# rneddojr/Adapting-Pretrained-Vision-Transformers-with-LoRA-against-Attack-Vectors

Hardware: AMD Instinct MI355X
Metric: adversarial images/sec (PGD-20, ViT-B/16+LoRA r=8, bs256) (higher is better)
Workload: dtype f16; 1 GPU; PGD-20 eps=8/255 alpha=2/255 random_start, ViT-B/16 (21 classes) + LoRA r=8 on q,k,v,attn-out,fc2 (fused), batch 256/GPU of synthetic 224x224x3 in HBM, seeded random-init weights; global_batch=256, per_gpu_batch=256, scaling=weak, pgd_steps=20, lora_rank=8, parallelism=dp1 (batch shards, no data-path collective), ranks_seen_by_collective=1

## Files before the change

adapting-pretrained-vision-transformers-with-lora-against-attack-vectors_amd/csrc/attention32.hip:

```cpp
#include <cstdlib>
#include <cstring>
#include <type_traits>

#include "env.h"
#include "kernels.h"
#include "prof.h"

namespace VLNS {

#ifdef VITLORA_ATTN_STAMPS
__device__ unsigned long long g_attn_stamps[8192 * 8 * 8];
#define STAMP(k) do { if (blockIdx.x < 8192 && (threadIdx.x & 63) == 0) g_attn_stamps[(blockIdx.x * 8 + (threadIdx.x >> 6)) * 8 + (k)] = __builtin_amdgcn_s_memtime(); } while (0)
#define ISTAMP(hd, k) do { if ((hd) == 3) { __builtin_amdgcn_sched_barrier(0); unsigned long long t_; asm volatile("s_memtime %0\n\ts_waitcnt lgkmcnt(0)" : "=s"(t_) :: "memory"); __builtin_amdgcn_sched_barrier(0); if (blockIdx.x < 1024 && (threadIdx.x & 63) == 0) g_attn_stamps[(blockIdx.x * 8 + (threadIdx.x >> 6)) * 8 + (k)] = t_; } } while (0)
#else
#define STAMP(k) do { } while (0)
#define ISTAMP(hd, k) do { } while (0)
#endif
#ifdef VITLORA_ATTN_STAMPS_FWD
#undef ISTAMP
#define ISTAMP(hd, k) do { } while (0)
#define FSTAMP(hd, k) do { if ((hd) == 3) { __builtin_amdgcn_sched_barrier(0); unsigned long long t_; asm volatile("s_memtime %0\n\ts_waitcnt lgkmcnt(0)" : "=s"(t_) :: "memory"); __builtin_amdgcn_sched_barrier(0); if (blockIdx.x < 1024 && (threadIdx.x & 63) == 0) g_attn_stamps[(blockIdx.x * 8 + (threadIdx.x >> 6)) * 8 + (k)] = t_; } } while (0)
#else
#define FSTAMP(hd, k) do { } while (0)
#endif
#ifdef VITLORA_ATTN_STAMPS2
#undef ISTAMP
#define ISTAMP(hd, k) do { } while (0)
#define JSTAMP(hd, i, k) do { if ((hd) == 3 && (i) == 3) { __builtin_amdgcn_sched_barrier(0); unsigned long long t_; asm volatile("s_memtime %0\n\ts_waitcnt lgkmcnt(0)" : "=s"(t_) :: "memory"); __builtin_amdgcn_sched_barrier(0); if (blockIdx.x < 1024 && (threadIdx.x & 63) == 0) g_attn_stamps[(blockIdx.x * 8 + (threadIdx.x >> 6)) * 8 + (k)] = t_; } } while (0)
#else
#define JSTAMP(hd, i, k) do { } while (0)
#endif

#define LDS_BARRIER()                                                        \
    do {                                                                     \
        __builtin_amdgcn_sched_barrier(0);                                   \
        asm volatile("s_waitcnt lgkmcnt(0)\n\ts_barrier" ::: "memory");       \
        __builtin_amdgcn_sched_barrier(0);                                   \
    } while (0)

namespace {

#ifndef VL_ATTN_NT
#define VL_ATTN_NT 0
#endif
__device__ __forceinline__ void glds16a(const void* gsrc, void* lds_wave_base) {
    __builtin_amdgcn_global_load_lds(GLB_PTR(gsrc), LDS_PTR(lds_wave_base), 16, 0, VL_ATTN_NT ? 2 : 0);
}
__device__ __forceinline__ h16x8 ld_attn(const h16* p) {
#if VL_ATTN_NT
    return __builtin_nontemporal_load((const h16x8*)p);
#else
    return *(const h16x8*)p;
#endif
}



constexpr int HD = 64;
#define TPAD(t) ((double)(((t) + 31) / 32 * 32))
typedef float f32x16 __attribute__((ext_vector_type(16)));
typedef float f32x2 __attribute__((ext_vector_type(2)));

__device__ __forceinline__ f32x16 mfma32(h16x8 a, h16x8 b, f32x16 c) {
#ifdef VL_BF16
    return __builtin_amdgcn_mfma_f32_32x32x16_bf16(a, b, c, 0, 0, 0);
#else
    return __builtin_amdgcn_mfma_f32_32x32x16_f16(a, b, c, 0, 0, 0);
#endif
}
__device__ __forceinline__ float fexp2(float x) { return __builtin_amdgcn_exp2f(x); }
__device__ __forceinline__ int swz(int r) { return (((r >> 1) & 1) << 2) | ((r >> 2) & 3); }

__device__ __forceinline__ h16x8 row_frag32(const h16* img, int row, int ks, int h) {
    return *(const h16x8*)(img + row * HD + (((2 * ks + h) ^ swz(row)) << 3));
}
__device__ __forceinline__ h16x8 tr_frag32(const h16* img, int t0, int c0, int lane) {
    const int g = lane >> 4, i = lane & 15;
    const int h = g >> 1, q = i >> 2, p = i & 3;
    const int col = c0 + 16 * (g & 1) + 4 * p;
    const int r0 = t0 + 4 * h + q, r1 = r0 + 8;
    const h16* a0 = img + r0 * HD + (((col >> 3) ^ swz(r0)) << 3) + (col & 4);
    const h16* a1 = img + r1 * HD + (((col >> 3) ^ swz(r1)) << 3) + (col & 4);
    return cat4(lds_read_tr16(a0), lds_read_tr16(a1));
}
__device__ __forceinline__ h16x8 pack8(const f32x16& v, int s) {
    h16x8 o;
#pragma unroll
    for (int j = 0; j < 8; ++j) o[j] = f2h(v[8 * s + j]);
    return o;
}
struct FragOffs {
    int row[4];
    int tr[2][2];
};
__device__ __forceinline__ FragOffs frag_offs(int lane) {
    FragOffs o;
    const int c = lane & 31, h = lane >> 5;
#pragma unroll
    for (int ks = 0; ks < 4; ++ks) o.row[ks] = c * HD + (((2 * ks + h) ^ swz(c)) << 3);
    const int g = lane >> 4, i = lane & 15;
    const int th = g >> 1, q = i >> 2, p = i & 3;
#pragma unroll
    for (int dt = 0; dt < 2; ++dt)
#pragma unroll
        for (int e = 0; e < 2; ++e) {
            const int r = 4 * th + q + 8 * e;
            o.tr[dt][e] = r * HD + (((dt * 4 + 2 * (g & 1) + (p >> 1)) ^ swz(r)) << 3) + ((p & 1) << 2);
        }
    return o;
}
__device__ __forceinline__ h16x8 row_frag_o(const h16* img, int tile, int off) {
    return *(const h16x8*)(img + tile * 32 * HD + off);
}
__device__ __forceinline__ h16x8 tr_frag_o(const h16* img, int tile, int st, const int (&off)[2]) {
    const h16* b = img + tile * 32 * HD + st * 16 * HD;
    return cat4(lds_read_tr16(b + off[0]), lds_read_tr16(b + off[1]));
}
template <int ROWS, int NW>
__device__ __forceinline__ void stage_glds(h16* img, const h16* src, int ld, int T, int w, int lane) {
    const int lr = lane >> 3, lc = lane & 7;
#pragma unroll 1
    for (int g = w; g < ROWS / 8; g += NW) {
        const int r = g * 8 + lr;
        const int rs = r < T ? r : T - 1;
        glds16a(src + (size_t)rs * ld + ((lc ^ swz(r)) << 3), img + g * 8 * HD);
    }
}

__device__ __forceinline__ void store_rows32_half(char* img, const f32x16 (&acc)[2], float mul, h16* dst0, int ld, int tok0,
                                                  int T, int lane) {
    const int c = lane & 31, h = lane >> 5;
    const int lr = lane >> 3, lc = lane & 7;
#pragma unroll
    for (int p = 0; p < 2; ++p) {
        if ((c >> 4) == p) {
#pragma unroll
            for (int dt = 0; dt < 2; ++dt)
#pragma unroll
                for (int rq = 0; rq < 4; ++rq) {
                    h16x4 o;
#pragma unroll
                    for (int k = 0; k < 4; ++k) o[k] = f2h(acc[dt][4 * rq + k] * mul);
                    *(h16x4*)(img + (c & 15) * 128 + (((dt * 4 + rq) ^ (c & 7)) << 4) + 8 * h) = o;
                }
        }
#pragma unroll
        for (int ps = 0; ps < 2; ++ps) {
            const int row = ps * 8 + lr;
            const h16x8 v = *(const h16x8*)(img + row * 128 + ((lc ^ lr) << 4));
            const int tok = tok0 + p * 16 + row;
            if (tok < T) *(h16x8*)(dst0 + (size_t)tok * ld + lc * 8) = v;
        }
    }
}

constexpr int FWD_WAVES = 8;
template <int NT>
__global__ __launch_bounds__(64 * FWD_WAVES) void attn_fwd32_kernel(const h16* __restrict__ qkv, h16* __restrict__ ctx,
                                                            float* __restrict__ lse2, int T, int H, int D, float scale_log2e) {
    constexpr int ROWS = NT * 32;
    __shared__ __attribute__((aligned(16))) h16 sm[2 * ROWS * HD];
    __shared__ __attribute__((aligned(16))) char wimg[FWD_WAVES * 2048];
    h16* sK = sm;
    h16* sV = sm + ROWS * HD;
    const int tid = threadIdx.x, lane = tid & 63;
    const int w = __builtin_amdgcn_readfirstlane(tid >> 6);
    const int c = lane & 31, h = lane >> 5;
    const int b = blockIdx.x / H, hd = blockIdx.x - b * H;
    const int ld = 3 * D;
    const h16* base = qkv + (size_t)b * T * ld + hd * HD;
    stage_glds<ROWS, FWD_WAVES>(sK, base + D, ld, T, w, lane);
    stage_glds<ROWS, FWD_WAVES>(sV, base + 2 * D, ld, T, w, lane);

    const int nqb = (T + 31) >> 5;
    int qb = w;
    h16x8 qf[4];
    auto load_q = [&](int blk) {
        const int q = blk * 32 + c;
        const h16* qr = base + (size_t)(q < T ? q : T - 1) * ld + 8 * h;
#pragma unroll
        for (int ks = 0; ks < 4; ++ks) qf[ks] = *(const h16x8*)(qr + 16 * ks);
    };
    if (qb < nqb) load_q(qb);
    asm volatile("s_waitcnt vmcnt(0)" ::: "memory");
    __syncthreads();

    const FragOffs fo = frag_offs(lane);
    const int tcut = T - 4 * h;
    for (; qb < nqb; qb += FWD_WAVES) {
        float m = -INFINITY, l = 0.f;
        f32x16 o[2];
#pragma unroll
        for (int dt = 0; dt < 2; ++dt)
#pragma unroll
            for (int r = 0; r < 16; ++r) o[dt][r] = 0.f;
        auto step = [&](int kt, auto masked) {
            constexpr bool MASKED = decltype(masked)::value;
            f32x16 s;
#pragma unroll
// ... 594 lines not shown
            auto stepA = [&](int kt, auto masked) {
                constexpr bool MASKED = decltype(masked)::value;
                f32x16 s, dp;
#pragma unroll
                for (int r = 0; r < 16; ++r) { s[r] = 0.f; dp[r] = 0.f; }
#pragma unroll
                for (int ks = 0; ks < 4; ++ks) {
                    s = mfma32(row_frag_o(sK, kt, fo.row[ks]), fa[ks], s);
                    dp = mfma32(row_frag_o(sV, kt, fo.row[ks]), fb[ks], dp);
                }
#pragma unroll
                for (int r = 0; r < 16; r += 2) {
                    const f32x2 t = f32x2{s[r], s[r + 1]} * f32x2{scale_log2e, scale_log2e} - f32x2{lse_q, lse_q};
                    f32x2 p = {fexp2(t[0]), fexp2(t[1])};
                    if constexpr (MASKED) {
                        if (kt * 32 + (r & 3) + 8 * (r >> 2) >= tcut) p[0] = 0.f;
                        if (kt * 32 + ((r + 1) & 3) + 8 * ((r + 1) >> 2) >= tcut) p[1] = 0.f;
                    }
                    const f32x2 d = p * (f32x2{dp[r], dp[r + 1]} - f32x2{delta_q, delta_q});
                    dp[r] = d[0]; dp[r + 1] = d[1];
                }
#pragma unroll
                for (int st = 0; st < 2; ++st) {
                    const h16x8 dsb = pack8(dp, st);
#pragma unroll
                    for (int dt = 0; dt < 2; ++dt) dq[dt] = mfma32(tr_frag_o(sK, kt, st, fo.tr[dt]), dsb, dq[dt]);
                }
            };
            const int nfull = T >> 5;
#pragma unroll 1
            for (int kt = 0; kt < nfull; ++kt) stepA(kt, std::false_type{});
            if (T & 31) stepA(nfull, std::true_type{});
            ISTAMP(hd, 1);
#pragma unroll
            for (int ks = 0; ks < 4; ++ks) { fa[ks] = row_frag32(sK, tok, ks, h); fb[ks] = row_frag32(sV, tok, ks, h); }
#pragma unroll
            for (int dt = 0; dt < 2; ++dt)
#pragma unroll
                for (int r = 0; r < 16; ++r) dq[dt][r] *= scale;
            if (lo.W && (lo.mods & 1u)) {
                f32x16 y;
#pragma unroll
                for (int r = 0; r < 16; ++r) y[r] = 0.f;
                const h16* sB = sBd + (hd & 1) * 3 * 8 * HD;
#pragma unroll
                for (int dt = 0; dt < 2; ++dt)
#pragma unroll
                    for (int st = 0; st < 2; ++st) y = mfma32(down_frag_lds(sB, dt, st, lane), pack8(dq[dt], st), y);
                down_accumulate(usum, y, tok, h);
            }
            store_rows32_half(wimg + w * 2048, dq, 1.f, dqkv + (size_t)b * T * ld + hd * HD, ld, w * 32, T, lane);
        }
        ISTAMP(hd, 2);
        LDS_BARRIER();
        ISTAMP(hd, 3);
        if (loader) {
            if (hd + 1 < H) {
                stage_glds<ROWS, 1>(sK, base + D + (hd + 1) * HD, ld, T, 0, lane);
                stage_glds<ROWS, 1>(sV, base + 2 * D + (hd + 1) * HD, ld, T, 0, lane);
                if (lo.W) stage_bd(hd + 1);
            }
            asm volatile("s_waitcnt vmcnt(0)" ::: "memory");
        } else if (active) {
            f32x16 dv[2], dk[2];
#pragma unroll
            for (int dt = 0; dt < 2; ++dt)
#pragma unroll
                for (int r = 0; r < 16; ++r) { dv[dt][r] = 0.f; dk[dt][r] = 0.f; }
#pragma unroll 1
            for (int qt = 0; qt < nb; ++qt) {
                f32x16 s, dp;
#pragma unroll
                for (int r = 0; r < 16; ++r) { s[r] = 0.f; dp[r] = 0.f; }
#pragma unroll
                for (int ks = 0; ks < 4; ++ks) {
                    s = mfma32(row_frag_o(sQ, qt, fo.row[ks]), fa[ks], s);
                    dp = mfma32(row_frag_o(sdO, qt, fo.row[ks]), fb[ks], dp);
                }
#pragma unroll
                for (int rq = 0; rq < 4; ++rq) {
                    const f32x4 lq = *(const f32x4*)(L + qt * 32 + 8 * rq + 4 * h);
                    const f32x4 dl = *(const f32x4*)(Dl + qt * 32 + 8 * rq + 4 * h);
#pragma unroll
                    for (int k = 0; k < 4; ++k) {
                        const float p = fexp2(fmaf(s[4 * rq + k], scale_log2e, -lq[k]));
                        s[4 * rq + k] = p;
                        dp[4 * rq + k] = p * (dp[4 * rq + k] - dl[k]);
                    }
                }
#pragma unroll
                for (int st = 0; st < 2; ++st) {
                    const h16x8 pb = pack8(s, st), dsb = pack8(dp, st);
#pragma unroll
                    for (int dt = 0; dt < 2; ++dt) {
                        dv[dt] = mfma32(tr_frag_o(sdO, qt, st, fo.tr[dt]), pb, dv[dt]);
                        dk[dt] = mfma32(tr_frag_o(sQ, qt, st, fo.tr[dt]), dsb, dk[dt]);
                    }
                }
            }
            ISTAMP(hd, 4);
#pragma unroll
            for (int dt = 0; dt < 2; ++dt)
#pragma unroll
                for (int r = 0; r < 16; ++r) dk[dt][r] *= scale;
            if (lo.W) {
                const h16* sB = sBd + (hd & 1) * 3 * 8 * HD;
#pragma unroll
                for (int md = 1; md < 3; ++md) {
                    if (!((lo.mods >> md) & 1u)) continue;
                    f32x16 y;
#pragma unroll
                    for (int r = 0; r < 16; ++r) y[r] = 0.f;
#pragma unroll
                    for (int dt = 0; dt < 2; ++dt)
#pragma unroll
                        for (int st = 0; st < 2; ++st)
                            y = mfma32(down_frag_lds(sB + md * 8 * HD, dt, st, lane), pack8(md == 1 ? dk[dt] : dv[dt], st), y);
                    down_accumulate(usum + md * ROWS * 8, y, tok, h);
                }
            }
            store_rows32_half(wimg + w * 2048, dk, 1.f, dqkv + (size_t)b * T * ld + D + hd * HD, ld, w * 32, T, lane);
            store_rows32_half(wimg + w * 2048, dv, 1.f, dqkv + (size_t)b * T * ld + 2 * D + hd * HD, ld, w * 32, T, lane);
            ISTAMP(hd, 7);
            if (hd + 1 < H) fetch_a(hd + 1);
        }
        ISTAMP(hd, 5);
        LDS_BARRIER();
        ISTAMP(hd, 6);
    }
    if (lo.W && !loader && active && tok < T && 4 * h < lo.r) {
        h16* dst = lo.out + ((size_t)b * T + tok) * 64 + 4 * h;
#pragma unroll
        for (int md = 0; md < 3; ++md) {
            if (!((lo.mods >> md) & 1u)) continue;
            const f32x4 u4 = *(const f32x4*)(usum + (md * ROWS + tok) * 8 + 4 * h);
            h16x4 v;
#pragma unroll
            for (int k = 0; k < 4; ++k) v[k] = f2h(u4[k]);
            *(h16x4*)(dst + md * lo.r) = v;
        }
    }
}

#ifndef RING_PRIO
#define RING_PRIO 0
#endif
template <int NT> constexpr int ring_img_rows() { return NT == 7 ? 200 : NT * 32; }
template <int NT>
size_t bwd_ring_lds() {
    return (size_t)4 * ring_img_rows<NT>() * HD * sizeof(h16) + (size_t)2 * NT * 2048 + (size_t)4 * NT * 32 * sizeof(float) +
           (size_t)3 * NT * 32 * 8 * sizeof(float) + (size_t)2 * 3 * 8 * HD * sizeof(h16);
}

template <int NT>
__global__ __launch_bounds__(64 * IMG_WAVES) void attn_bwd_ring_kernel(const h16* __restrict__ qkv, const h16* __restrict__ ctx,
                                                                       const h16* __restrict__ dctx, const float* __restrict__ lse2,
                                                                       h16* __restrict__ dqkv, int T, int H, int D, float scale,
                                                                       float scale_log2e, const LoraDown lo) {
    constexpr int ROWS = NT * 32, IR = ring_img_rows<NT>();
    extern __shared__ __attribute__((aligned(16))) char smem[];
    h16* sQ = (h16*)smem;
    h16* sdO = sQ + IR * HD;
    h16* sK0 = sdO + IR * HD;
    char* sE = (char*)(sK0 + 2 * IR * HD);
    float* sLD = (float*)(sE + 2 * NT * 2048);
    float* usum = sLD + 4 * ROWS;
    h16* sBd = (h16*)(usum + 3 * ROWS * 8);

    const int tid = threadIdx.x, lane = tid & 63;
    const int w = __builtin_amdgcn_readfirstlane(tid >> 6);
    const int c = lane & 31, h = lane >> 5;
    const int b = blockIdx.x;
    const int ld = 3 * D;
    const h16* base = qkv + (size_t)b * T * ld;
    const h16* dobase = dctx + (size_t)b * T * D;
    const h16* obase = ctx + (size_t)b * T * D;
    const int nb = (T + 31) >> 5;

    for (int i = tid; i < 3 * ROWS * 8; i += 64 * IMG_WAVES) usum[i] = 0.f;
    for (int i = tid; i < 2 * NT * 2048 / 16; i += 64 * IMG_WAVES) ((f32x4*)sE)[i] = f32x4{0.f, 0.f, 0.f, 0.f};
    if constexpr (ROWS > IR)
        for (int i = tid; i < (ROWS - IR) * HD * 2 / 16; i += 64 * IMG_WAVES) ((f32x4*)(sK0 + IR * HD))[i] = f32x4{0.f, 0.f, 0.f, 0.f};

    if (w == IMG_WAVES - 1) {
        h16x8 bdv[3];
        auto bd_issue = [&](int hd) {
            const int j = lane >> 3, c8 = (lane & 7) * 8;
#pragma unroll
            for (int md = 0; md < 3; ++md) {
#pragma unroll
                for (int k = 0; k < 8; ++k) bdv[md][k] = (h16)0.f;
                if (((lo.mods >> md) & 1u) && j < lo.r) bdv[md] = *(const h16x8*)(lo.W + (size_t)(md * lo.r + j) * ld + md * D + hd * HD + c8);
            }
        };
        auto bd_commit = [&](int hd) {
            const int j = lane >> 3, c8 = (lane & 7) * 8;
            h16* dst = sBd + (hd & 1) * 3 * 8 * HD;
#pragma unroll
            for (int md = 0; md < 3; ++md) *(h16x8*)(dst + md * 8 * HD + j * HD + c8) = bdv[md];
        };
        h16x8 rd8[4], ro8[4];
        float rlse = 0.f;
        auto consts_issue = [&](int hd, int blk) {
            const int t = blk * 32 + c, tc = t < T ? t : T - 1;
#pragma unroll
            for (int ks = 0; ks < 4; ++ks) {
                rd8[ks] = ld_attn(dobase + (size_t)tc * D + hd * HD + 8 * h + 16 * ks);
                ro8[ks] = ld_attn(obase + (size_t)tc * D + hd * HD + 8 * h + 16 * ks);
            }
            rlse = lse2[((size_t)b * H + hd) * T + tc];
        };
        auto consts_finish = [&](int hd, int blk) {
            const int t = blk * 32 + c;
            float delta_q = 0.f;
#pragma unroll
            for (int ks = 0; ks < 4; ++ks)
#pragma unroll
                for (int k = 0; k < 8; ++k) delta_q = fmaf(h2f(rd8[ks][k]), h2f(ro8[ks][k]), delta_q);
            delta_q += __shfl_xor(delta_q, 32, 64);
            if (h == 0) {
                float* Lw = sLD + (hd & 1) * 2 * ROWS;
                Lw[t] = t < T ? rlse : INFINITY;
                Lw[ROWS + t] = t < T ? delta_q : 0.f;
            }
        };
        stage_glds<IR, 1>(sQ, base, ld, T, 0, lane);
        stage_glds<IR, 1>(sdO, dobase, D, T, 0, lane);
        stage_glds<IR, 1>(sK0, base + D, ld, T, 0, lane);
        if (lo.W) {
            h16x8 z;
#pragma unroll
            for (int k = 0; k < 8; ++k) z[k] = (h16)0.f;
            for (int i = lane; i < T * 8; i += 64) *(h16x8*)(lo.out + ((size_t)b * T + (i >> 3)) * 64 + (i & 7) * 8) = z;
            bd_issue(0);
            bd_commit(0);
        }
        for (int blk = 0; blk < NT; ++blk) { consts_issue(0, blk); consts_finish(0, blk); }
        asm volatile("s_waitcnt vmcnt(0)" ::: "memory");
        LDS_BARRIER();
#pragma unroll 1
        for (int hd = 0; hd < H; ++hd) {
            const bool more = hd + 1 < H;
            ISTAMP(hd, 0);
            if (more) {
                consts_issue(hd + 1, 0);
                if (lo.W) bd_issue(hd + 1);
            }
#pragma unroll 1
            for (int i = 0; i < nb; ++i) {
                if (i == 3) ISTAMP(hd, 1);
                if (more) {
                    consts_finish(hd + 1, i);
                    if (i == 0 && lo.W) bd_commit(hd + 1);
                    if (i + 1 < NT) consts_issue(hd + 1, i + 1);
                    {
                        constexpr int NG = IR / 8;
                        const int per = (NG + nb - 1) / nb;
                        const int lr = lane >> 3, lc = lane & 7;
                        h16* img = sK0 + ((hd + 1) & 1) * IR * HD;
                        const h16* src = base + D + (hd + 1) * HD;
                        for (int g = i * per; g < (i + 1) * per && g < NG; ++g) {
                            const int r = g * 8 + lr;
                            const int rs = r < T ? r : T - 1;
                            glds16a(src + (size_t)rs * ld + ((lc ^ swz(r)) << 3), img + g * 8 * HD);
                        }
                    }
                }
                if (i == nb - 1) {
                    if (more) for (int blk = nb; blk < NT; ++blk) { consts_finish(hd + 1, blk); if (blk + 1 < NT) consts_issue(hd + 1, blk + 1); }
                    asm volatile("s_waitcnt vmcnt(0)" ::: "memory");
                }
                if (i == 3) ISTAMP(hd, 2);
                LDS_BARRIER();
                if (i == 3) ISTAMP(hd, 3);
            }
            ISTAMP(hd, 4);
            if (more) {
                stage_glds<IR, 1>(sQ, base + (hd + 1) * HD, ld, T, 0, lane);
                stage_glds<IR, 1>(sdO, dobase + (hd + 1) * HD, D, T, 0, lane);
            }
            asm volatile("s_waitcnt vmcnt(0)" ::: "memory");
            ISTAMP(hd, 6);
            LDS_BARRIER();
            ISTAMP(hd, 7);
        }
        return;
    }
    if (w >= nb) {
        LDS_BARRIER();
        for (int hd = 0; hd < H; ++hd) {
            for (int i = 0; i < nb; ++i) LDS_BARRIER();
            LDS_BARRIER();
        }
        return;
    }
    const FragOffs fo = frag_offs(lane);
    const int tok = w * 32 + c, tokc = tok < T ? tok : T - 1;
    int ewr[2], erd[2];
    {
        const int f = (c >> 2) & 3;
#pragma unroll
        for (int r1 = 0; r1 < 2; ++r1) ewr[r1] = c * 64 + (((2 * r1 + h) ^ f) << 3);
        const int g = lane >> 4, i16 = lane & 15, q4 = i16 >> 2, p4 = i16 & 3;
#pragma unroll
        for (int e = 0; e < 2; ++e) {
            const int r = 4 * (g >> 1) + q4 + 8 * e;
            erd[e] = r * 64 + (((4 * (g & 1) + p4) ^ ((r >> 2) & 3)) << 3);
        }
    }
    h16x8 fb[4];
#pragma unroll
    for (int ks = 0; ks < 4; ++ks) fb[ks] = ld_attn(base + (size_t)tokc * ld + 2 * D + 8 * h + 16 * ks);
    if (w >= 4 && RING_PRIO) __builtin_amdgcn_s_setprio(1);
    LDS_BARRIER();

#pragma unroll 1
    for (int hd = 0; hd < H; ++hd) {
        const h16* sK = sK0 + (hd & 1) * IR * HD;
        const float* L = sLD + (hd & 1) * 2 * ROWS;
        const float* Dl = L + ROWS;
        f32x16 dq[2], dk[2], dv[2];
#pragma unroll
        for (int dt = 0; dt < 2; ++dt)
#pragma unroll
            for (int r = 0; r < 16; ++r) { dq[dt][r] = 0.f; dk[dt][r] = 0.f; dv[dt][r] = 0.f; }
        h16x8 pbk[2], dsk[2];
#pragma unroll
        for (int st = 0; st < 2; ++st)
#pragma unroll
            for (int j = 0; j < 8; ++j) { pbk[st][j] = (h16)0.f; dsk[st][j] = (h16)0.f; }
        int qp = w, kp = w;
        ISTAMP(hd, 0);
        auto take_ds = [&](int step, int kt_, int st) -> h16x8 {
            const char* eslot = sE + ((step & 1) * NT + w) * 2048;
            h16x8 d = cat4(lds_read_tr16(eslot + 1024 * st + erd[0]), lds_read_tr16(eslot + 1024 * st + erd[1]));
            if (kt_ == nb - 1 && (T & 31)) {
#pragma unroll
                for (int j = 0; j < 8; ++j)
                    if (kt_ * 32 + 16 * st + 8 * (j >> 2) + 4 * h + (j & 3) >= T) d[j] = (h16)0.f;
            }
            return d;
        };
#pragma unroll 1
        for (int i = 0; i < nb; ++i) {
            int qt = w + i; if (qt >= nb) qt -= nb;
            int kt = w - i; if (kt < 0) kt += nb;
            if (i == 3) ISTAMP(hd, 1);
            JSTAMP(hd, i, 0);
            f32x16 s, dp;
#pragma unroll
            for (int r = 0; r < 16; ++r) { s[r] = 0.f; dp[r] = 0.f; }
#pragma unroll
            for (int ks = 0; ks < 4; ++ks) s = mfma32(row_frag_o(sQ, qt, fo.row[ks]), row_frag_o(sK, w, fo.row[ks]), s);
#pragma unroll
            for (int ks = 0; ks < 4; ++ks) dp = mfma32(row_frag_o(sdO, qt, fo.row[ks]), fb[ks], dp);
            h16x8 fv0[2], fk0[2], fv1[2], fk1[2], fq0[2], fq1[2], d0, d1;
#pragma unroll
            for (int dt = 0; dt < 2; ++dt) { fv0[dt] = tr_frag_o(sdO, qp, 0, fo.tr[dt]); fk0[dt] = tr_frag_o(sQ, qp, 0, fo.tr[dt]); }
            __builtin_amdgcn_sched_barrier(0);
            JSTAMP(hd, i, 1);
            char* eslot_w = sE + ((i & 1) * NT + qt) * 2048;
            auto exp_piece = [&](int rq) {
                const f32x4 lq = *(const f32x4*)(L + qt * 32 + 8 * rq + 4 * h);
                const f32x4 dl = *(const f32x4*)(Dl + qt * 32 + 8 * rq + 4 * h);
                h16x4 ds4;
#pragma unroll
                for (int k = 0; k < 4; ++k) {
                    const float p = fexp2(fmaf(s[4 * rq + k], scale_log2e, -lq[k]));
                    const float d = p * (dp[4 * rq + k] - dl[k]);
                    pbk[rq >> 1][4 * (rq & 1) + k] = f2h(p);
                    ds4[k] = f2h_sat(d);
                    dsk[rq >> 1][4 * (rq & 1) + k] = ds4[k];
                }
                *(h16x4*)(eslot_w + ewr[rq & 1] + 32 * (rq >> 1)) = ds4;
            };
#pragma unroll
            for (int dt = 0; dt < 2; ++dt) { fv1[dt] = tr_frag_o(sdO, qp, 1, fo.tr[dt]); fk1[dt] = tr_frag_o(sQ, qp, 1, fo.tr[dt]); }
#pragma unroll
            for (int dt = 0; dt < 2; ++dt) { dv[dt] = mfma32(fv0[dt], pbk[0], dv[dt]); dk[dt] = mfma32(fk0[dt], dsk[0], dk[dt]); }
            exp_piece(0);
            __builtin_amdgcn_sched_barrier(0);
            JSTAMP(hd, i, 2);
            d0 = take_ds(i + 1, kp, 0);
#pragma unroll
            for (int dt = 0; dt < 2; ++dt) fq0[dt] = tr_frag_o(sK, kp, 0, fo.tr[dt]);
#pragma unroll
            for (int dt = 0; dt < 2; ++dt) { dv[dt] = mfma32(fv1[dt], pbk[1], dv[dt]); dk[dt] = mfma32(fk1[dt], dsk[1], dk[dt]); }
            exp_piece(1);
            __builtin_amdgcn_sched_barrier(0);
            JSTAMP(hd, i, 3);
            d1 = take_ds(i + 1, kp, 1);
#pragma unroll
            for (int dt = 0; dt < 2; ++dt) fq1[dt] = tr_frag_o(sK, kp, 1, fo.tr[dt]);
            if (i == 0) {
#pragma unroll
                for (int j = 0; j < 8; ++j) { d0[j] = (h16)0.f; d1[j] = (h16)0.f; }
            }
#pragma unroll
            for (int dt = 0; dt < 2; ++dt) dq[dt] = mfma32(fq0[dt], d0, dq[dt]);
            exp_piece(2);
            __builtin_amdgcn_sched_barrier(0);
            JSTAMP(hd, i, 4);
#pragma unroll
            for (int dt = 0; dt < 2; ++dt) dq[dt] = mfma32(fq1[dt], d1, dq[dt]);
            exp_piece(3);
            __builtin_amdgcn_sched_barrier(0);
            JSTAMP(hd, i, 5);
            qp = qt; kp = kt;
            if (i == nb - 1) {
#pragma unroll
                for (int st = 0; st < 2; ++st)
#pragma unroll
                    for (int dt = 0; dt < 2; ++dt) {
                        dv[dt] = mfma32(tr_frag_o(sdO, qp, st, fo.tr[dt]), pbk[st], dv[dt]);
                        dk[dt] = mfma32(tr_frag_o(sQ, qp, st, fo.tr[dt]), dsk[st], dk[dt]);
                    }
            }
            if (i == 3) ISTAMP(hd, 2);
            JSTAMP(hd, i, 6);
            LDS_BARRIER();
            if (i == 3) ISTAMP(hd, 3);
            JSTAMP(hd, i, 7);
        }
        ISTAMP(hd, 4);
#pragma unroll
        for (int st = 0; st < 2; ++st) {
            const h16x8 d = take_ds(nb - 1, kp, st);
#pragma unroll
            for (int dt = 0; dt < 2; ++dt) dq[dt] = mfma32(tr_frag_o(sK, kp, st, fo.tr[dt]), d, dq[dt]);
        }
        {
            int ln = lane;
            asm volatile("" : "+v"(ln));
            const int c2 = ln & 31, h2 = ln >> 5, tok2 = w * 32 + c2, tokc2 = tok2 < T ? tok2 : T - 1;
            if (hd + 1 < H) {
#pragma unroll
                for (int ks = 0; ks < 4; ++ks) fb[ks] = ld_attn(base + (size_t)tokc2 * ld + 2 * D + (hd + 1) * HD + 8 * h2 + 16 * ks);
            }
#pragma unroll
            for (int dt = 0; dt < 2; ++dt)
#pragma unroll
                for (int r = 0; r < 16; ++r) { dq[dt][r] *= scale; dk[dt][r] *= scale; }
            if (lo.W) {
                const h16* sB = sBd + (hd & 1) * 3 * 8 * HD;
#pragma unroll
                for (int md = 0; md < 3; ++md) {
                    if (!((lo.mods >> md) & 1u)) continue;
                    f32x16 y;
#pragma unroll
                    for (int r = 0; r < 16; ++r) y[r] = 0.f;
#pragma unroll
                    for (int dt = 0; dt < 2; ++dt)
#pragma unroll
                        for (int st = 0; st < 2; ++st)
                            y = mfma32(down_frag_lds(sB + md * 8 * HD, dt, st, ln), pack8(md == 0 ? dq[dt] : md == 1 ? dk[dt] : dv[dt], st), y);
                    down_accumulate(usum + md * ROWS * 8, y, tok2, h2);
                }
            }
            ISTAMP(hd, 5);
            char* wimg = sE + ((nb & 1) * NT + w) * 2048;
            h16* drow = dqkv + (size_t)b * T * ld + hd * HD;
            store_rows32_half(wimg, dq, 1.f, drow, ld, w * 32, T, ln);
            store_rows32_half(wimg, dk, 1.f, drow + D, ld, w * 32, T, ln);
            store_rows32_half(wimg, dv, 1.f, drow + 2 * D, ld, w * 32, T, ln);
        }
        ISTAMP(hd, 6);
        LDS_BARRIER();
        ISTAMP(hd, 7);
    }
    if (lo.W && tok < T && 4 * h < lo.r) {
        h16* dst = lo.out + ((size_t)b * T + tok) * 64 + 4 * h;
#pragma unroll
        for (int md = 0; md < 3; ++md) {
            if (!((lo.mods >> md) & 1u)) continue;
            const f32x4 u4 = *(const f32x4*)(usum + (md * ROWS + tok) * 8 + 4 * h);
            h16x4 v;
#pragma unroll
            for (int k = 0; k < 4; ++k) v[k] = f2h(u4[k]);
            *(h16x4*)(dst + md * lo.r) = v;
        }
    }
}

template <int NT>
void launch_fwd_img(const h16* qkv, h16* ctx, float* lse2, int B, int T, int H, int D, const LoraDown& lo, hipStream_t s) {
    const float sl = 0.125f * 1.4426950408889634f;
    hipLaunchKernelGGL((attn_fwd_img_kernel<NT>), dim3(B), dim3(64 * IMG_WAVES), fwd_img_lds<NT>(), s, qkv, ctx, lse2, T, H, D, sl, lo);
}
int g_attn_ring = 1;
template <int NT>
void launch_bwd_img(const h16* qkv, const h16* ctx, const h16* dctx, const float* lse2, h16* dqkv, int B, int T, int H, int D,
                    const LoraDown& lo, bool ring, hipStream_t s) {
    const float scale = 0.125f;
    if (ring) {
        hipLaunchKernelGGL((attn_bwd_ring_kernel<NT>), dim3(B), dim3(64 * IMG_WAVES), bwd_ring_lds<NT>(), s, qkv, ctx, dctx, lse2, dqkv,
                           T, H, D, scale, scale * 1.4426950408889634f, lo);
        return;
    }
    hipLaunchKernelGGL((attn_bwd_img_kernel<NT>), dim3(B), dim3(64 * IMG_WAVES), bwd_img_lds<NT>(), s, qkv, ctx, dctx, lse2, dqkv,
                       T, H, D, scale, scale * 1.4426950408889634f, lo);
}

template <int NT>
size_t bwd_lds() { return (size_t)4 * NT * 32 * HD * sizeof(h16) + (size_t)2 * NT * 32 * sizeof(float); }

template <int NT>
void launch_bwd(const h16* qkv, const h16* ctx, const h16* dctx, const float* lse2, h16* dqkv, int B, int T, int H,
                int D, hipStream_t s) {
    const float scale = 0.125f;
    hipLaunchKernelGGL((attn_bwd32_kernel<NT>), dim3(B * H), dim3(512), bwd_lds<NT>(), s, qkv, ctx, dctx, lse2, dqkv, T,
                       H, D, scale, scale * 1.4426950408889634f);
}

}

void attention32_set_ring(int on) { g_attn_ring = on ? 1 : 0; }

int attention32_init(int device) {
    static bool done[64] = {};
    if (device < 0 || device >= 64) return -1;
    if (done[device]) return 0;
    hipError_t e = hipFuncSetAttribute((const void*)attn_bwd32_kernel<1>, hipFuncAttributeMaxDynamicSharedMemorySize, (int)bwd_lds<1>());
    if (e != hipSuccess) return (int)e;
    e = hipFuncSetAttribute((const void*)attn_bwd32_kernel<7>, hipFuncAttributeMaxDynamicSharedMemorySize, (int)bwd_lds<7>());
    if (e != hipSuccess) return (int)e;
    e = hipFuncSetAttribute((const void*)attn_fwd_img_kernel<1>, hipFuncAttributeMaxDynamicSharedMemorySize, (int)fwd_img_lds<1>());
    if (e != hipSuccess) return (int)e;
    e = hipFuncSetAttribute((const void*)attn_fwd_img_kernel<7>, hipFuncAttributeMaxDynamicSharedMemorySize, (int)fwd_img_lds<7>());
    if (e != hipSuccess) return (int)e;
    e = hipFuncSetAttribute((const void*)attn_bwd_img_kernel<1>, hipFuncAttributeMaxDynamicSharedMemorySize, (int)bwd_img_lds<1>());
    if (e != hipSuccess) return (int)e;
    e = hipFuncSetAttribute((const void*)attn_bwd_img_kernel<7>, hipFuncAttributeMaxDynamicSharedMemorySize, (int)bwd_img_lds<7>());
    if (e != hipSuccess) return (int)e;
    e = hipFuncSetAttribute((const void*)attn_bwd_ring_kernel<1>, hipFuncAttributeMaxDynamicSharedMemorySize, (int)bwd_ring_lds<1>());
    if (e != hipSuccess) return (int)e;
    e = hipFuncSetAttribute((const void*)attn_bwd_ring_kernel<7>, hipFuncAttributeMaxDynamicSharedMemorySize, (int)bwd_ring_lds<7>());
    if (e != hipSuccess) return (int)e;
    g_attn_ring = env_flag("VITLORA_ATTN_RING", g_attn_ring != 0);
    done[device] = true;
    return 0;
}

int k_attention32_fwd(const h16* qkv, h16* ctx, float* lse2, int B, int T, int H, int D, hipStream_t s) {
    ProfScope prof_("attn_fwd32_kernel", 4.0 * B * H * (double)T * T * HD, (double)B * T * D * 8.0, s, 4.0 * B * H * (double)TPAD(T) * TPAD(T) * HD);
    const float sl = 0.125f * 1.4426950408889634f;
    if (T <= 32) hipLaunchKernelGGL((attn_fwd32_kernel<1>), dim3(B * H), dim3(64 * FWD_WAVES), 0, s, qkv, ctx, lse2, T, H, D, sl);
    else if (T <= 224) hipLaunchKernelGGL((attn_fwd32_kernel<7>), dim3(B * H), dim3(64 * FWD_WAVES), 0, s, qkv, ctx, lse2, T, H, D, sl);
    else return -1;
    return 0;
}

int k_attention32_bwd(const h16* qkv, const h16* ctx, const h16* dctx, const float* lse2, h16* dqkv, int B, int T,
                      int H, int D, hipStream_t s) {
    ProfScope prof_("attn_bwd32_kernel", 10.0 * B * H * (double)T * T * HD, (double)B * T * D * 16.0, s, 10.0 * B * H * (double)TPAD(T) * TPAD(T) * HD);
    if (T <= 32) launch_bwd<1>(qkv, ctx, dctx, lse2, dqkv, B, T, H, D, s);
    else if (T <= 224) launch_bwd<7>(qkv, ctx, dctx, lse2, dqkv, B, T, H, D, s);
    else return -1;
    return 0;
}

int k_attention_img_fwd(const h16* qkv, h16* ctx, float* lse2, int B, int T, int H, int D, const h16* Ad, h16* t, int r,
                        hipStream_t s) {
    ProfScope prof_("attn_fwd_img_kernel", 4.0 * B * H * (double)T * T * HD, (double)B * T * D * 8.0, s, 4.0 * B * H * (double)TPAD(T) * TPAD(T) * HD);
    LoraDown lo;
    lo.W = Ad; lo.out = t; lo.r = r; lo.mods = 1u;
    if (!Ad || !t || r <= 0 || r > 8) { lo.W = nullptr; lo.out = nullptr; }
    if (T <= 32) launch_fwd_img<1>(qkv, ctx, lse2, B, T, H, D, lo, s);
    else if (T <= 224) launch_fwd_img<7>(qkv, ctx, lse2, B, T, H, D, lo, s);
    else return -1;
    return 0;
}
int k_attention_img_bwd(const h16* qkv, const h16* ctx, const h16* dctx, const float* lse2, h16* dqkv, int B, int T, int H, int D,
                        const h16* Bd, h16* u, int r, unsigned mods, hipStream_t s, int force_ring) {
    const int ring_rows = T <= 32 ? ring_img_rows<1>() : ring_img_rows<7>();
    if (force_ring == 1 && T > ring_rows) return -1;
    const bool ring = force_ring >= 0 ? force_ring == 1 : g_attn_ring && T <= ring_rows;
    ProfScope prof_(ring ? "attn_bwd_ring_kernel" : "attn_bwd_img_kernel", 10.0 * B * H * (double)T * T * HD, (double)B * T * D * 16.0, s,
                    (ring ? 10.0 : 14.0) * B * H * (double)TPAD(T) * TPAD(T) * HD);
    LoraDown lo;
    lo.W = Bd; lo.out = u; lo.r = r; lo.mods = mods;
    if (!Bd || !u || r <= 0 || r > 8 || !mods) { lo.W = nullptr; lo.out = nullptr; }
    if (T <= 32) launch_bwd_img<1>(qkv, ctx, dctx, lse2, dqkv, B, T, H, D, lo, ring, s);
    else if (T <= 224) launch_bwd_img<7>(qkv, ctx, dctx, lse2, dqkv, B, T, H, D, lo, ring, s);
    else return -1;
    return 0;
}

}
```

Baseline: 507.2 img/s.

## Restructure attention-backward producer wave with inline-asm loads and register-staged prefetch

The producer wave in the ring attention-backward kernel now issues its global loads through inline asm with precise vmcnt waits, and unrolls the per-block loop at compile time. When every wave has work, part of the next head's Q/dO tiles are staged through registers and written to LDS after the loop, instead of all going through LDS-DMA at the end. The head-0 row constants (lse and delta) are now computed by the compute waves themselves rather than serially by the producer. The aim is to shorten the producer's critical path between barriers and overlap more prefetch with compute, at the cost of fragile hand-counted vmcnt values and higher register pressure.

```diff
diff --git a/adapting-pretrained-vision-transformers-with-lora-against-attack-vectors_amd/csrc/attention32.hip b/adapting-pretrained-vision-transformers-with-lora-against-attack-vectors_amd/csrc/attention32.hip
--- a/adapting-pretrained-vision-transformers-with-lora-against-attack-vectors_amd/csrc/attention32.hip
+++ b/adapting-pretrained-vision-transformers-with-lora-against-attack-vectors_amd/csrc/attention32.hip
@@ -1,6 +1,7 @@
 #include <cstdlib>
 #include <cstring>
 #include <type_traits>
+#include <utility>
 
 #include "env.h"
 #include "kernels.h"
@@ -12,9 +13,12 @@
 __device__ unsigned long long g_attn_stamps[8192 * 8 * 8];
 #define STAMP(k) do { if (blockIdx.x < 8192 && (threadIdx.x & 63) == 0) g_attn_stamps[(blockIdx.x * 8 + (threadIdx.x >> 6)) * 8 + (k)] = __builtin_amdgcn_s_memtime(); } while (0)
 #define ISTAMP(hd, k) do { if ((hd) == 3) { __builtin_amdgcn_sched_barrier(0); unsigned long long t_; asm volatile("s_memtime %0\n\ts_waitcnt lgkmcnt(0)" : "=s"(t_) :: "memory"); __builtin_amdgcn_sched_barrier(0); if (blockIdx.x < 1024 && (threadIdx.x & 63) == 0) g_attn_stamps[(blockIdx.x * 8 + (threadIdx.x >> 6)) * 8 + (k)] = t_; } } while (0)
+__device__ unsigned long long g_attn_clock[1024 * 4];
+#define CSTAMP(k) do { if (blockIdx.x < 1024 && threadIdx.x == 0) { g_attn_clock[blockIdx.x * 4 + (k)] = __builtin_amdgcn_s_memtime(); g_attn_clock[blockIdx.x * 4 + (k) + 1] = __builtin_amdgcn_s_memrealtime(); } } while (0)
 #else
 #define STAMP(k) do { } while (0)
 #define ISTAMP(hd, k) do { } while (0)
+#define CSTAMP(k) do { } while (0)
 #endif
 #ifdef VITLORA_ATTN_STAMPS_FWD
 #undef ISTAMP
@@ -45,6 +49,37 @@
 #endif
 __device__ __forceinline__ void glds16a(const void* gsrc, void* lds_wave_base) {
     __builtin_amdgcn_global_load_lds(GLB_PTR(gsrc), LDS_PTR(lds_wave_base), 16, 0, VL_ATTN_NT ? 2 : 0);
+}
+template <int IMM = 0>
+__device__ __forceinline__ f32x4 ring_gload16(const void* sbase, unsigned voff) {
+    f32x4 v;
+    asm volatile("global_load_dwordx4 %0, %1, %2 offset:%3" : "=&v"(v) : "v"(voff), "s"(sbase), "n"(IMM) : "memory");
+    return v;
+}
+__device__ __forceinline__ float ring_gload4(const void* sbase, unsigned voff) {
+    float v;
+    asm volatile("global_load_dword %0, %1, %2" : "=&v"(v) : "v"(voff), "s"(sbase) : "memory");
+    return v;
+}
+template <int N>
+__device__ __forceinline__ void ring_wait(f32x4 (&a)[4], f32x4 (&b)[4], float& c) {
+    asm volatile("s_waitcnt vmcnt(%9)"
+                 : "+v"(a[0]), "+v"(a[1]), "+v"(a[2]), "+v"(a[3]), "+v"(b[0]), "+v"(b[1]), "+v"(b[2]), "+v"(b[3]), "+v"(c)
+                 : "n"(N) : "memory");
+}
+template <int N>
+__device__ __forceinline__ void ring_wait_bd(f32x4 (&a)[3]) {
+    asm volatile("s_waitcnt vmcnt(%3)" : "+v"(a[0]), "+v"(a[1]), "+v"(a[2]) : "n"(N) : "memory");
+}
+template <int N, int NS>
+__device__ __forceinline__ void ring_wait_all(f32x4 (&a)[NS]) {
+    asm volatile("s_waitcnt vmcnt(%0)" ::"n"(N) : "memory");
+#pragma unroll
+    for (int g = 0; g < NS; ++g) asm volatile("" : "+v"(a[g]));
+}
+template <int... I, class F>
+__device__ __forceinline__ void ring_static_for(std::integer_sequence<int, I...>, F&& f) {
+    (f(std::integral_constant<int, I>{}), ...);
 }
 __device__ __forceinline__ h16x8 ld_attn(const h16* p) {
 #if VL_ATTN_NT
@@ -945,6 +980,31 @@
            (size_t)3 * NT * 32 * 8 * sizeof(float) + (size_t)2 * 3 * 8 * HD * sizeof(h16);
 }
 
+template <int NT> constexpr int ring_staged_groups() { return 2 * (ring_img_rows<NT>() / 8); }
+constexpr int ring_slice(int n, int per, int j) {
+    const int a = j * per < n ? j * per : n, b = (j + 1) * per < n ? (j + 1) * per : n;
+    return b - a;
+}
+__device__ __forceinline__ void ring_glds16(const void* sbase, unsigned voff, const void* lds_wave_base) {
+    const unsigned lds_addr = (unsigned)(size_t)(__attribute__((address_space(3))) const char*)lds_wave_base;
+    unsigned keep;
+    asm volatile("s_mov_b32 %0, m0\n\ts_mov_b32 m0, %3\n\ts_nop 0\n\tglobal_load_lds_dwordx4 %1, %2\n\ts_mov_b32 m0, %0"
+                 : "=&s"(keep) : "v"(voff), "s"(sbase), "s"(lds_addr) : "memory");
+}
+__device__ __forceinline__ void ring_row_consts(float* Lw, int rows, const h16x8 (&d8)[4], const h16x8 (&o8)[4], float lse, int t,
+                                                int T, int h) {
+    float delta_q = 0.f;
+#pragma unroll
+    for (int ks = 0; ks < 4; ++ks)
+#pragma unroll
+        for (int k = 0; k < 8; ++k) delta_q = fmaf(h2f(d8[ks][k]), h2f(o8[ks][k]), delta_q);
+    delta_q += __shfl_xor(delta_q, 32, 64);
+    if (h == 0) {
+        Lw[t] = t < T ? lse : INFINITY;
+        Lw[rows + t] = t < T ? delta_q : 0.f;
+    }
+}
+
 template <int NT>
 __global__ __launch_bounds__(64 * IMG_WAVES) void attn_bwd_ring_kernel(const h16* __restrict__ qkv, const h16* __restrict__ ctx,
                                                                        const h16* __restrict__ dctx, const float* __restrict__ lse2,
@@ -976,110 +1036,175 @@
         for (int i = tid; i < (ROWS - IR) * HD * 2 / 16; i += 64 * IMG_WAVES) ((f32x4*)(sK0 + IR * HD))[i] = f32x4{0.f, 0.f, 0.f, 0.f};
 
     if (w == IMG_WAVES - 1) {
-        h16x8 bdv[3];
+        constexpr int NG = IR / 8;
+        constexpr int NS = ring_staged_groups<NT>();
+        constexpr int PERK = (NG + NT - 1) / NT, PERS = (NS + NT - 1) / NT;
+        static_assert(NS <= 2 * NG && 3 + 2 * (9 + PERK + PERS) <= 63, "vmcnt counts at most 63 operations");
+        auto lane_now = [&] { int ln = lane; asm volatile("" : "+v"(ln)); return ln; };
+        f32x4 stg[NS];
+        f32x4 bdv[3];
         auto bd_issue = [&](int hd) {
-            const int j = lane >> 3, c8 = (lane & 7) * 8;
+            const int ln = lane_now(), lr = ln >> 3, lc = ln & 7;
+            const h16* wb = (lo.W ? lo.W : qkv) + hd * HD;
 #pragma unroll
             for (int md = 0; md < 3; ++md) {
-#pragma unroll
-                for (int k = 0; k < 8; ++k) bdv[md][k] = (h16)0.f;
-                if (((lo.mods >> md) & 1u) && j < lo.r) bdv[md] = *(const h16x8*)(lo.W + (size_t)(md * lo.r + j) * ld + md * D + hd * HD + c8);
+                const bool on = lo.W && ((lo.mods >> md) & 1u) && lr < lo.r;
+                bdv[md] = ring_gload16(wb, on ? (unsigned)(((md * lo.r + lr) * ld + md * D + lc * 8) * 2) : 0u);
             }
         };
         auto bd_commit = [&](int hd) {
-            const int j = lane >> 3, c8 = (lane & 7) * 8;
             h16* dst = sBd + (hd & 1) * 3 * 8 * HD;
-#pragma unroll
-            for (int md = 0; md < 3; ++md) *(h16x8*)(dst + md * 8 * HD + j * HD + c8) = bdv[md];
+            const int ln = lane_now(), lr = ln >> 3, lc = ln & 7;
+#pragma unroll
+            for (int md = 0; md < 3; ++md) {
+                const bool on = ((lo.mods >> md) & 1u) && lr < lo.r;
+                *(f32x4*)(dst + md * 8 * HD + lr * HD + lc * 8) = on ? bdv[md] : f32x4{0.f, 0.f, 0.f, 0.f};
+            }
         };
-        h16x8 rd8[4], ro8[4];
+        f32x4 rd8[4], ro8[4];
         float rlse = 0.f;
         auto consts_issue = [&](int hd, int blk) {
-            const int t = blk * 32 + c, tc = t < T ? t : T - 1;
-#pragma unroll
-            for (int ks = 0; ks < 4; ++ks) {
-                rd8[ks] = ld_attn(dobase + (size_t)tc * D + hd * HD + 8 * h + 16 * ks);
-                ro8[ks] = ld_attn(obase + (size_t)tc * D + hd * HD + 8 * h + 16 * ks);
-            }
-            rlse = lse2[((size_t)b * H + hd) * T + tc];
+            const int ln = lane_now(), t = blk * 32 + (ln & 31), tc = t < T ? t : T - 1;
+            const unsigned off = (unsigned)((tc * D + 8 * (ln >> 5)) * 2);
+            const h16* sd = dobase + hd * HD;
+            const h16* so = obase + hd * HD;
+            rd8[0] = ring_gload16<0>(sd, off); rd8[1] = ring_gload16<32>(sd, off);
+            rd8[2] = ring_gload16<64>(sd, off); rd8[3] = ring_gload16<96>(sd, off);
+            ro8[0] = ring_gload16<0>(so, off); ro8[1] = ring_gload16<32>(so, off);
+            ro8[2] = ring_gload16<64>(so, off); ro8[3] = ring_gload16<96>(so, off);
+            rlse = ring_gload4(lse2 + ((size_t)b * H + hd) * T, (unsigned)(tc * 4));
         };
         auto consts_finish = [&](int hd, int blk) {
-            const int t = blk * 32 + c;
-            float delta_q = 0.f;
-#pragma unroll
-            for (int ks = 0; ks < 4; ++ks)
-#pragma unroll
-                for (int k = 0; k < 8; ++k) delta_q = fmaf(h2f(rd8[ks][k]), h2f(ro8[ks][k]), delta_q);
-            delta_q += __shfl_xor(delta_q, 32, 64);
-            if (h == 0) {
-                float* Lw = sLD + (hd & 1) * 2 * ROWS;
-                Lw[t] = t < T ? rlse : INFINITY;
-                Lw[ROWS + t] = t < T ? delta_q : 0.f;
-            }
+            h16x8 d8[4], o8[4];
+#pragma unroll
+            for (int ks = 0; ks < 4; ++ks) { d8[ks] = __builtin_bit_cast(h16x8, rd8[ks]); o8[ks] = __builtin_bit_cast(h16x8, ro8[ks]); }
+            const int ln = lane_now();
+            ring_row_consts(sLD + (hd & 1) * 2 * ROWS, ROWS, d8, o8, rlse, blk * 32 + (ln & 31), T, ln >> 5);
         };
-        stage_glds<IR, 1>(sQ, base, ld, T, 0, lane);
-        stage_glds<IR, 1>(sdO, dobase, D, T, 0, lane);
-        stage_glds<IR, 1>(sK0, base + D, ld, T, 0, lane);
+        auto grp_off = [&](int ln, int g, int ldx) {
+            const int r = g * 8 + (ln >> 3), rs = r < T ? r : T - 1;
+            return (unsigned)((rs * ldx + (((ln & 7) ^ swz(r)) << 3)) * 2);
+        };
+        auto img_dma = [&](h16* img, const h16* src, int ldx, int g0, int g1) {
+            const int ln = lane_now();
+#pragma unroll 1
+            for (int g = g0; g < g1; ++g) ring_glds16(src, grp_off(ln, g, ldx), img + g * 8 * HD);
+        };
+        auto stage_issue = [&](int hd, auto s0c, auto s1c) {
+            constexpr int S0 = decltype(s0c)::value, S1 = decltype(s1c)::value;
+            const h16* sq = base + hd * HD;
+            const h16* sd = dobase + hd * HD;
+            const int ln = lane_now();
+#pragma unroll
+            for (int s = S0; s < S1; ++s) {
+                if (s < NG) stg[s] = ring_gload16(sq, grp_off(ln, s, ld));
+                else stg[s] = ring_gload16(sd, grp_off(ln, s - NG, D));
+            }
+        };
+        auto issue_slice = [&](int hd, auto jc, auto fullc) {
+            constexpr int j = decltype(jc)::value;
+            constexpr int k0 = j * PERK < NG ? j * PERK : NG, k1 = (j + 1) * PERK < NG ? (j + 1) * PERK : NG;
+            constexpr int s0 = j * PERS < NS ? j * PERS : NS, s1 = (j + 1) * PERS < NS ? (j + 1) * PERS : NS;
+            consts_issue(hd, j);
+            const int ln = lane_now();
+#pragma unroll
+            for (int g = k0; g < k1; ++g) ring_glds16(base + D + hd * HD, grp_off(ln, g, ld), sK0 + (hd & 1) * IR * HD + g * 8 * HD);
+            if constexpr (decltype(fullc)::value) stage_issue(hd, std::integral_constant<int, s0>{}, std::integral_constant<int, s1>{});
+        };
+        img_dma(sQ, base, ld, 0, NG);
+        img_dma(sdO, dobase, D, 0, NG);
+        img_dma(sK0, base + D, ld, 0, NG);
         if (lo.W) {
             h16x8 z;
 #pragma unroll
             for (int k = 0; k < 8; ++k) z[k] = (h16)0.f;
             for (int i = lane; i < T * 8; i += 64) *(h16x8*)(lo.out + ((size_t)b * T + (i >> 3)) * 64 + (i & 7) * 8) = z;
-            bd_issue(0);
-            bd_commit(0);
-        }
-        for (int blk = 0; blk < NT; ++blk) { consts_issue(0, blk); consts_finish(0, blk); }
+        }
+        bd_issue(0);
+        ring_wait_bd<0>(bdv);
+        if (lo.W) bd_commit(0);
         asm volatile("s_waitcnt vmcnt(0)" ::: "memory");
+        __builtin_amdgcn_s_waitcnt(0x0f70);
         LDS_BARRIER();
+        auto run_heads = [&](auto fullc) {
+            constexpr bool FULL = decltype(fullc)::value;
+            constexpr int NSE = FULL ? NS : 0;
 #pragma unroll 1
-        for (int hd = 0; hd < H; ++hd) {
-            const bool more = hd + 1 < H;
-            ISTAMP(hd, 0);
-            if (more) {
-                consts_issue(hd + 1, 0);
-                if (lo.W) bd_issue(hd + 1);
-            }
+            for (int hd = 0; hd < H; ++hd) {
+                const bool more = hd + 1 < H;
+                ISTAMP(hd, 0);
+                if (more) {
+                    bd_issue(hd + 1);
+                    issue_slice(hd + 1, std::integral_constant<int, 0>{}, fullc);
+                    ring_static_for(std::make_integer_sequence<int, NT>{}, [&](auto ic) {
+                        constexpr int i = decltype(ic)::value;
+                        if (FULL || i < nb) {
+                            if (i == 3) ISTAMP(hd, 1);
+                            constexpr int younger = ring_slice(NG, PERK, i) + ring_slice(NSE, PERS, i);
+                            ring_wait<younger>(rd8, ro8, rlse);
+                            consts_finish(hd + 1, i);
+                            if constexpr (i == 0) {
+                                ring_wait_bd<younger>(bdv);
+                                if (lo.W) bd_commit(hd + 1);
+                            }
+                            if constexpr (i + 1 < NT) {
+                                if (FULL || i + 1 < nb) {
+                                    issue_slice(hd + 1, std::integral_constant<int, i + 1>{}, fullc);
+                                } else {
+                                    constexpr int k0 = (i + 1) * PERK < NG ? (i + 1) * PERK : NG;
+                                    img_dma(sK0 + ((hd + 1) & 1) * IR * HD, base + D + (hd + 1) * HD, ld, k0, NG);
+                                    if (h == 0) {
+                                        float* Lw = sLD + ((hd + 1) & 1) * 2 * ROWS;
+                                        for (int t = (i + 1) * 32 + c; t < ROWS; t += 32) { Lw[t] = INFINITY; Lw[ROWS + t] = 0.f; }
+                                    }
+                                }
+                            }
+                            if (i == 3) ISTAMP(hd, 2);
+                            LDS_BARRIER();
+                            if (i == 3) ISTAMP(hd, 3);
+                        }
+                    });
+                } else {
 #pragma unroll 1
-            for (int i = 0; i < nb; ++i) {
-                if (i == 3) ISTAMP(hd, 1);
+                    for (int i = 0; i < nb; ++i) {
+                        if (i == 3) ISTAMP(hd, 1);
+                        if (i == 3) ISTAMP(hd, 2);
+                        LDS_BARRIER();
+                        if (i == 3) ISTAMP(hd, 3);
+                    }
+                }
+                ISTAMP(hd, 4);
                 if (more) {
-                    consts_finish(hd + 1, i);
-                    if (i == 0 && lo.W) bd_commit(hd + 1);
-                    if (i + 1 < NT) consts_issue(hd + 1, i + 1);
-                    {
-                        constexpr int NG = IR / 8;
-                        const int per = (NG + nb - 1) / nb;
-                        const int lr = lane >> 3, lc = lane & 7;
-                        h16* img = sK0 + ((hd + 1) & 1) * IR * HD;
-                        const h16* src = base + D + (hd + 1) * HD;
-                        for (int g = i * per; g < (i + 1) * per && g < NG; ++g) {
-                            const int r = g * 8 + lr;
-                            const int rs = r < T ? r : T - 1;
-                            glds16a(src + (size_t)rs * ld + ((lc ^ swz(r)) << 3), img + g * 8 * HD);
+                    if constexpr (FULL) {
+                        const int ln = lane_now();
+#pragma unroll
+                        for (int s = NS; s < 2 * NG; ++s) {
+                            if (s < NG) ring_glds16(base + (hd + 1) * HD, grp_off(ln, s, ld), sQ + s * 8 * HD);
+                            else ring_glds16(dobase + (hd + 1) * HD, grp_off(ln, s - NG, D), sdO + (s - NG) * 8 * HD);
                         }
+                        ring_wait_all<2 * NG - NS>(stg);
+#pragma unroll
+                        for (int s = 0; s < NS; ++s) *(f32x4*)((s < NG ? sQ + s * 8 * HD : sdO + (s - NG) * 8 * HD) + ln * 8) = stg[s];
+                    } else {
+                        img_dma(sQ, base + (hd + 1) * HD, ld, 0, NG);
+                        img_dma(sdO, dobase + (hd + 1) * HD, D, 0, NG);
                     }
                 }
-                if (i == nb - 1) {
-                    if (more) for (int blk = nb; blk < NT; ++blk) { consts_finish(hd + 1, blk); if (blk + 1 < NT) consts_issue(hd + 1, blk + 1); }
-                    asm volatile("s_waitcnt vmcnt(0)" ::: "memory");
-                }
-                if (i == 3) ISTAMP(hd, 2);
+                asm volatile("s_waitcnt vmcnt(0)" ::: "memory");
+                ISTAMP(hd, 6);
                 LDS_BARRIER();
-                if (i == 3) ISTAMP(hd, 3);
-            }
-            ISTAMP(hd, 4);
-            if (more) {
-                stage_glds<IR, 1>(sQ, base + (hd + 1) * HD, ld, T, 0, lane);
-                stage_glds<IR, 1>(sdO, dobase + (hd + 1) * HD, D, T, 0, lane);
-            }
-            asm volatile("s_waitcnt vmcnt(0)" ::: "memory");
-            ISTAMP(hd, 6);
-            LDS_BARRIER();
-            ISTAMP(hd, 7);
-        }
+                ISTAMP(hd, 7);
+            }
+        };
+        if (NT == 1 || nb == NT) run_heads(std::true_type{});
+        else if constexpr (NT > 1) run_heads(std::false_type{});
         return;
     }
     if (w >= nb) {
+        if (h == 0 && w < NT) {
+            sLD[w * 32 + c] = INFINITY;
+            sLD[ROWS + w * 32 + c] = 0.f;
+        }
         LDS_BARRIER();
         for (int hd = 0; hd < H; ++hd) {
             for (int i = 0; i < nb; ++i) LDS_BARRIER();
@@ -1104,8 +1229,18 @@
     h16x8 fb[4];
 #pragma unroll
     for (int ks = 0; ks < 4; ++ks) fb[ks] = ld_attn(base + (size_t)tokc * ld + 2 * D + 8 * h + 16 * ks);
+    {
+        h16x8 d8[4], o8[4];
+#pragma unroll
+        for (int ks = 0; ks < 4; ++ks) {
+            d8[ks] = ld_attn(dobase + (size_t)tokc * D + 8 * h + 16 * ks);
+            o8[ks] = ld_attn(obase + (size_t)tokc * D + 8 * h + 16 * ks);
+        }
+        ring_row_consts(sLD, ROWS, d8, o8, lse2[(size_t)b * H * T + tokc], tok, T, h);
+    }
     if (w >= 4 && RING_PRIO) __builtin_amdgcn_s_setprio(1);
     LDS_BARRIER();
+    CSTAMP(0);
 
 #pragma unroll 1
     for (int hd = 0; hd < H; ++hd) {
@@ -1261,6 +1396,7 @@
         LDS_BARRIER();
         ISTAMP(hd, 7);
     }
+    CSTAMP(2);
     if (lo.W && tok < T && 4 * h < lo.r) {
         h16* dst = lo.out + ((size_t)b * T + tok) * 64 + 4 * h;
 #pragma unroll
```

Measured after the change: 508.9 img/s (median of 6 runs). No clear change (+0.3%).
